# mormj/newsched

Measured on NVIDIA B200. Metric: Msamples/s FIR-ccf & FFT-4096 flowgraph at 1/2/4/8 B200; % of HBM/FP32 roofline, higher is better.
Workload: dtype f32

## Files before the change

### newsched_b200/csrc/common.cuh

```cuda
#pragma once
#include <cuda.h>
#include <cuda_runtime.h>
#include <atomic>
#include <cstdarg>
#include <cstdint>
#include <cstdio>
#include <cstring>

#include "../../include/b200dsp.h"

namespace b200 {

char* err_buf();
int set_err(int code, const char* fmt, ...);
extern std::atomic<int64_t> g_launches;

inline cudaStream_t cs(b200_stream_t s) { return reinterpret_cast<cudaStream_t>(s); }

#define B200_CUDA(call)                                                                  \
    do {                                                                                 \
        cudaError_t e__ = (call);                                                        \
        if (e__ != cudaSuccess)                                                          \
            return ::b200::set_err(B200_ERR_CUDA, "%s:%d %s -> %s", __FILE__, __LINE__,  \
                                   #call, cudaGetErrorString(e__));                      \
    } while (0)

#define B200_LAUNCH(kernel, grid, block, smem, stream, ...)                              \
    do {                                                                                 \
        kernel<<<(grid), (block), (smem), (stream)>>>(__VA_ARGS__);                      \
        ::b200::g_launches.fetch_add(1, std::memory_order_relaxed);                      \
        cudaError_t e__ = cudaPeekAtLastError();                                         \
        if (e__ != cudaSuccess)                                                          \
            return ::b200::set_err(B200_ERR_CUDA, "%s:%d launch %s -> %s", __FILE__,     \
                                   __LINE__, #kernel, cudaGetErrorString(e__));          \
    } while (0)

#define B200_LAUNCH_PDL(kernel, grid_, block_, smem_, stream_, ...)                          \
    do {                                                                                 \
        cudaLaunchConfig_t cfg__{};                                                      \
        cfg__.gridDim = dim3(grid_);                                                     \
        cfg__.blockDim = dim3(block_);                                                   \
        cfg__.dynamicSmemBytes = (smem_);                                                \
        cfg__.stream = (stream_);                                                        \
        cudaLaunchAttribute attr__[1];                                                   \
        attr__[0].id = cudaLaunchAttributeProgrammaticStreamSerialization;               \
        attr__[0].val.programmaticStreamSerializationAllowed = 1;                        \
        cfg__.attrs = attr__;                                                            \
        cfg__.numAttrs = 1;                                                              \
        cudaError_t e__ = cudaLaunchKernelEx(&cfg__, kernel, __VA_ARGS__);               \
        ::b200::g_launches.fetch_add(1, std::memory_order_relaxed);                      \
        if (e__ != cudaSuccess)                                                          \
            return ::b200::set_err(B200_ERR_CUDA, "%s:%d launch %s -> %s", __FILE__,     \
                                   __LINE__, #kernel, cudaGetErrorString(e__));          \
    } while (0)

__device__ __forceinline__ void pdl_wait() { asm volatile("griddepcontrol.wait;" ::: "memory"); }
__device__ __forceinline__ void pdl_launch_dependents() { asm volatile("griddepcontrol.launch_dependents;" ::: "memory"); }

int sm_count();

typedef CUresult (*tmap_encode_fn)(CUtensorMap*, CUtensorMapDataType, cuuint32_t, void*, const cuuint64_t*,
                                   const cuuint64_t*, const cuuint32_t*, const cuuint32_t*, CUtensorMapInterleave,
                                   CUtensorMapSwizzle, CUtensorMapL2promotion, CUtensorMapFloatOOBfill);
tmap_encode_fn tmap_encode_tiled();

__device__ __forceinline__ float2 cmul_nofma(float2 a, float kre, float kim)
{
    float ac = __fmul_rn(a.x, kre), bd = __fmul_rn(a.y, kim);
    float ad = __fmul_rn(a.x, kim), bc = __fmul_rn(a.y, kre);
    return make_float2(__fsub_rn(ac, bd), __fadd_rn(ad, bc));
}

#ifndef B200_PK_CMUL
#define B200_PK_CMUL 0
#endif
__device__ __forceinline__ float2 cmul(float2 a, float2 b)
{
#if B200_PK_CMUL
    const float2 r = __fmul2_rn(b, make_float2(a.x, a.x));
    return __ffma2_rn(make_float2(-b.y, b.x), make_float2(a.y, a.y), r);
#else
    return make_float2(fmaf(-a.y, b.y, a.x * b.x), fmaf(a.x, b.y, a.y * b.x));
#endif
}
__device__ __forceinline__ float2 cmul_conj(float2 a, float2 b)
{
#if B200_PK_CMUL
    const float2 r = __fmul2_rn(make_float2(b.x, -b.y), make_float2(a.x, a.x));
    return __ffma2_rn(make_float2(b.y, b.x), make_float2(a.y, a.y), r);
#else
    return make_float2(fmaf(a.y, b.y, a.x * b.x), fmaf(-a.x, b.y, a.y * b.x));
#endif
}
__device__ __forceinline__ float2 cmac(float2 a, float2 b, float2 acc)
{
#if B200_PK_CMUL
    acc = __ffma2_rn(b, make_float2(a.x, a.x), acc);
    return __ffma2_rn(make_float2(-b.y, b.x), make_float2(a.y, a.y), acc);
#else
    return make_float2(fmaf(a.x, b.x, fmaf(-a.y, b.y, acc.x)), fmaf(a.x, b.y, fmaf(a.y, b.x, acc.y)));
#endif
}

__device__ __forceinline__ float mag_nofma(float2 a)
{
    return __fsqrt_rn(__fadd_rn(__fmul_rn(a.x, a.x), __fmul_rn(a.y, a.y)));
}

__device__ __forceinline__ uint32_t smem_u32(const void* p)
{
    return (uint32_t)__cvta_generic_to_shared(p);
}
__device__ __forceinline__ void mbar_init(uint64_t* bar, uint32_t count)
{
    asm volatile("mbarrier.init.shared::cta.b64 [%0], %1;" ::"r"(smem_u32(bar)), "r"(count) : "memory");
}
__device__ __forceinline__ void fence_mbar_init()
{
    asm volatile("fence.mbarrier_init.release.cluster;" ::: "memory");
}
__device__ __forceinline__ void fence_proxy_async()
{
    asm volatile("fence.proxy.async.shared::cta;" ::: "memory");
}
__device__ __forceinline__ void mbar_arrive_expect_tx(uint64_t* bar, uint32_t bytes)
{
    asm volatile("mbarrier.arrive.expect_tx.shared::cta.b64 _, [%0], %1;" ::"r"(smem_u32(bar)), "r"(bytes)
                 : "memory");
}
__device__ __forceinline__ void bulk_copy_g2s(void* smem_dst, const void* gmem_src, uint32_t bytes,
                                              uint64_t* bar)
{
    asm volatile("cp.async.bulk.shared::cluster.global.mbarrier::complete_tx::bytes [%0], [%1], %2, [%3];" ::"r"(
                     smem_u32(smem_dst)),
                 "l"(gmem_src), "r"(bytes), "r"(smem_u32(bar))
                 : "memory");
}
__device__ __forceinline__ bool mbar_try_wait(uint64_t* bar, uint32_t parity)
{
    uint32_t ok;
    asm volatile("{\n"
                 ".reg .pred p;\n"
                 "mbarrier.try_wait.parity.shared::cta.b64 p, [%1], %2;\n"
                 "selp.u32 %0, 1, 0, p;\n"
                 "}"
                 : "=r"(ok)
                 : "r"(smem_u32(bar)), "r"(parity)
                 : "memory");
    return ok != 0;
}
__device__ __forceinline__ void mbar_wait(uint64_t* bar, uint32_t parity)
{
    for (uint32_t spins = 0; !mbar_try_wait(bar, parity); spins++)
        if (spins > (1u << 28))
            __trap();
}

}
```

### newsched_b200/csrc/fft.cu

```cuda
#include <cmath>
#include <cstdlib>
#include <vector>

#include "fft_core.cuh"

#ifndef B200_FFT_TW2
#define B200_FFT_TW2 1
#endif

namespace b200 {

template <bool FWD, int OUT>
__global__ void __launch_bounds__(256, 2)
    fft4096_kernel(const float2* __restrict__ in, void* __restrict__ out, long long n_vec,
                   const float* __restrict__ weff, const float2* __restrict__ tw1,
                   const float2* __restrict__ tw2)
{
    __shared__ float2 sA[16 * F4K_STRIDE];
    __shared__ float2 sT2[256];
    const int tid = threadIdx.x;

    float wreg[16];
    float2 t1[16];
#pragma unroll
    for (int i = 0; i < 16; i++) {
        wreg[i] = __ldg(weff + i * 256 + tid);
        t1[i] = __ldg(tw1 + i * 256 + tid);
    }
    sT2[tid] = __ldg(tw2 + tid);
    __syncthreads();

    for (long long vec = blockIdx.x; vec < n_vec; vec += gridDim.x) {
        const float2* x = in + vec * 4096;
        float2 v[16];
        if (tid == 0 && vec + gridDim.x < n_vec && ((uintptr_t)in % 16 == 0))
            asm volatile("cp.async.bulk.prefetch.L2.global [%0], %1;" ::"l"(in + (vec + gridDim.x) * 4096),
                         "r"(4096 * 8)
                         : "memory");
#pragma unroll
        for (int i = 0; i < 16; i++)
            v[i] = __ldcs(x + i * 256 + tid);
#pragma unroll
        for (int i = 0; i < 16; i++)
            v[i] = __fmul2_rn(v[i], make_float2(wreg[i], wreg[i]));
        dft16<FWD>(v);
#pragma unroll
        for (int k0 = 0; k0 < 16; k0++)
            sA[k0 * F4K_STRIDE + tid] = cmul(v[pos16(k0)], t1[k0]);
        __syncthreads();
        {
            const int k0 = tid >> 4, n0 = tid & 15;
            float2* row = sA + k0 * F4K_STRIDE + n0;
#pragma unroll
            for (int i = 0; i < 16; i++)
                v[i] = row[i * 16];
            dft16<FWD>(v);
            row[0] = v[pos16(0)];
#pragma unroll
            for (int k1 = 1; k1 < 16; k1++)
                row[k1 * 16] = cmul(v[pos16(k1)], sT2[k1 * 16 + n0]);
        }
        __syncthreads();
        {
            const int k0 = tid & 15, k1 = tid >> 4;
            const float2* row = sA + k0 * F4K_STRIDE + k1 * 16;
#pragma unroll
            for (int i = 0; i < 16; i++)
                v[i] = row[i];
            dft16<FWD>(v);
            if (OUT == B200_FFT_OUT_COMPLEX) {
                float2* y = reinterpret_cast<float2*>(out) + vec * 4096;
#pragma unroll
                for (int k2 = 0; k2 < 16; k2++)
                    __stcs(y + k2 * 256 + tid, v[pos16(k2)]);
            } else {
                float* y = reinterpret_cast<float*>(out) + vec * 4096;
#pragma unroll
                for (int k2 = 0; k2 < 16; k2++) {
                    float2 z = v[pos16(k2)];
                    float p = fmaf(z.x, z.x, z.y * z.y);
                    __stcs(y + k2 * 256 + tid, OUT == B200_FFT_OUT_MAG ? sqrt_approx(p) : p);
                }
            }
        }
        __syncthreads();
    }
}

constexpr int f4k_ntile(int out) { return out == B200_FFT_OUT_COMPLEX ? 2 : 3; }
constexpr size_t f4k_tma_smem(int out) { return (size_t)f4k_ntile(out) * (4096 * 8 + 8) + 256 * 8; }

__device__ __forceinline__ int f4k_swz(int n0, int k0) { return (((n0 >> 1) ^ (k0 & 7)) << 1) | (n0 & 1); }

template <bool FWD, int OUT>
__global__ void __launch_bounds__(256, 2)
    fft4096_tma_kernel(const float2* __restrict__ in, void* __restrict__ out, long long n_vec,
                       const float* __restrict__ weff, const float2* __restrict__ tw1,
                       const float2* __restrict__ tw2)
{
    constexpr int NT = f4k_ntile(OUT);
    extern __shared__ __align__(128) unsigned char smem_raw[];
    float2* sTile0 = reinterpret_cast<float2*>(smem_raw);
    float2* sT2 = sTile0 + 4096 * NT;
    uint64_t* bar0 = reinterpret_cast<uint64_t*>(sT2 + 256);
    const int tid = threadIdx.x;

    if (tid == 0) {
#pragma unroll
        for (int i = 0; i < NT; i++)
            mbar_init(bar0 + i, 1);
        fence_mbar_init();
    }
    float wreg[16];
    float2 t1[16];
#pragma unroll
    for (int i = 0; i < 16; i++) {
        wreg[i] = __ldg(weff + i * 256 + tid);
        t1[i] = __ldg(tw1 + i * 256 + tid);
    }
    sT2[tid] = __ldg(tw2 + tid);
    __syncthreads();
#if B200_FFT_TW2 == 1
    float2 t2r[16];
#pragma unroll
    for (int k1 = 1; k1 < 16; k1++)
        t2r[k1] = sT2[k1 * 16 + (tid & 15)];
#endif
    pdl_wait();
    pdl_launch_dependents();
    long long vec = blockIdx.x;
    if (tid == 0) {
#pragma unroll
        for (int i = 0; i < NT - 1; i++)
            if (vec + (long long)i * gridDim.x < n_vec) {
                mbar_arrive_expect_tx(bar0 + i, 4096 * 8);
                bulk_copy_g2s(sTile0 + 4096 * i, in + (vec + (long long)i * gridDim.x) * 4096, 4096 * 8, bar0 + i);
            }
    }
    int t = 0;
    uint32_t par = 0;
    for (; vec < n_vec; vec += gridDim.x) {
        float2 v[16];
        float2* tile = sTile0 + t * 4096;
        mbar_wait(bar0 + t, par);
#pragma unroll
        for (int i = 0; i < 16; i++)
            v[i] = tile[i * 256 + tid];
#pragma unroll
        for (int i = 0; i < 16; i++)
            v[i] = __fmul2_rn(v[i], make_float2(wreg[i], wreg[i]));
        dft16<FWD>(v);
#pragma unroll
        for (int k0 = 0; k0 < 16; k0++)
            tile[k0 * 256 + tid] = cmul(v[pos16(k0)], t1[k0]);
#if B200_FFT_TW2 == 2
        float2 t2r[16];
#pragma unroll
        for (int k1 = 1; k1 < 16; k1++)
            t2r[k1] = sT2[k1 * 16 + (tid & 15)];
#endif
        __syncthreads();
        const int tn = t == 0 ? NT - 1 : t - 1;
        if (tid == 0 && vec + (long long)(NT - 1) * gridDim.x < n_vec) {
            fence_proxy_async();
            mbar_arrive_expect_tx(bar0 + tn, 4096 * 8);
            bulk_copy_g2s(sTile0 + tn * 4096, in + (vec + (long long)(NT - 1) * gridDim.x) * 4096, 4096 * 8,
                          bar0 + tn);
        }
        {
            const int k0 = tid >> 4, n0 = tid & 15;
            float2* row = tile + k0 * 256;
#pragma unroll
            for (int i = 0; i < 16; i++)
                v[i] = row[i * 16 + n0];
            __syncwarp();
            dft16<FWD>(v);
            float2* dst = row + f4k_swz(n0, k0);
            dst[0] = v[pos16(0)];
#pragma unroll
            for (int k1 = 1; k1 < 16; k1++)
#if B200_FFT_TW2
                dst[k1 * 16] = cmul(v[pos16(k1)], t2r[k1]);
#else
                dst[k1 * 16] = cmul(v[pos16(k1)], sT2[k1 * 16 + n0]);
#endif
        }
        __syncthreads();
        {
            const int k0 = tid & 15, k1 = tid >> 4, s = k0 & 7;
            const float4* seg = reinterpret_cast<const float4*>(tile + k0 * 256 + k1 * 16);
#pragma unroll
            for (int j = 0; j < 8; j++) {
                const float4 q = seg[j ^ s];
                v[2 * j] = make_float2(q.x, q.y);
                v[2 * j + 1] = make_float2(q.z, q.w);
            }
            dft16<FWD>(v);
            if (OUT == B200_FFT_OUT_COMPLEX) {
                float2* y = reinterpret_cast<float2*>(out) + vec * 4096;
#pragma unroll
                for (int k2 = 0; k2 < 16; k2++)
                    __stcs(y + k2 * 256 + tid, v[pos16(k2)]);
            } else {
                float* y = reinterpret_cast<float*>(out) + vec * 4096;
#pragma unroll
                for (int k2 = 0; k2 < 16; k2++) {
                    float2 z = v[pos16(k2)];
                    float p = fmaf(z.x, z.x, z.y * z.y);
                    __stcs(y + k2 * 256 + tid, OUT == B200_FFT_OUT_MAG ? sqrt_approx(p) : p);
                }
            }
        }
        if (++t == NT) {
            t = 0;
            par ^= 1;
        }
    }
}

#ifndef B200_F8K_EARLY
#define B200_F8K_EARLY 0
#endif
constexpr size_t F8K_SMEM = 8192 * 8 + 16 * F4K_STRIDE * 8 + 256 * 8 + 32;

template <bool FWD, int I>
__device__ __forceinline__ float2 mul_w32(float2 z)
{
    constexpr double kPi = 3.14159265358979323846;
    constexpr float cr[16] = { 1.f, 0.98078528040323043f, 0.92387953251128674f, 0.83146961230254524f,
                               0.70710678118654752f, 0.55557023301960218f, 0.38268343236508977f,
                               0.19509032201612825f, 0.f, -0.19509032201612825f, -0.38268343236508977f,
                               -0.55557023301960218f, -0.70710678118654752f, -0.83146961230254524f,
                               -0.92387953251128674f, -0.98078528040323043f };
    constexpr float si[16] = { 0.f, 0.19509032201612825f, 0.38268343236508977f, 0.55557023301960218f,
                               0.70710678118654752f, 0.83146961230254524f, 0.92387953251128674f,
                               0.98078528040323043f, 1.f, 0.98078528040323043f, 0.92387953251128674f,
                               0.83146961230254524f, 0.70710678118654752f, 0.55557023301960218f,
                               0.38268343236508977f, 0.19509032201612825f };
    (void)kPi;
    if (I == 0)
        return z;
    constexpr float wr = cr[I], wi = FWD ? -si[I] : si[I];
    return make_float2(fmaf(-z.y, wi, z.x * wr), fmaf(z.x, wi, z.y * wr));
}

template <bool FWD, int I = 0>
__device__ __forceinline__ void f8k_split(float2 (&a)[16], float2* sIn, const float* __restrict__ w0,
                                          const float* __restrict__ w1, float2 wt, int tid)
{
    if constexpr (I < 16) {
        const float2 x0 = __fmul2_rn(sIn[I * 256 + tid], make_float2(w0[I], w0[I]));
        const float2 x1 = __fmul2_rn(sIn[4096 + I * 256 + tid], make_float2(w1[I], w1[I]));
        a[I] = x0 + x1;
        sIn[I * 256 + tid] = cmul(mul_w32<FWD, I>(x0 - x1), wt);
        f8k_split<FWD, I + 1>(a, sIn, w0, w1, wt, tid);
    }
}

template <bool FWD, int OUT>
__global__ void __launch_bounds__(256, 2)
    fft8192_kernel(const float2* __restrict__ in, void* __restrict__ out, long long n_vec,
                   const float* __restrict__ weff, const float2* __restrict__ tw1,
                   const float2* __restrict__ tw2, float odd_sign)
{
    extern __shared__ __align__(128) unsigned char smem_raw[];
    float2* sIn = reinterpret_cast<float2*>(smem_raw);
    float2* sA = sIn + 8192;
    float2* sT2 = sA + 16 * F4K_STRIDE;
    uint64_t* bar = reinterpret_cast<uint64_t*>(sT2 + 256);
    const int tid = threadIdx.x;
    if (tid == 0) {
        mbar_init(bar, 1);
        mbar_init(bar + 1, 1);
        fence_mbar_init();
    }
    float2 t1[16];
#pragma unroll
    for (int i = 0; i < 16; i++)
        t1[i] = __ldg(tw1 + i * 256 + tid);
    sT2[tid] = __ldg(tw2 + tid);
    float2 wt;
    {
        float sn, cs_;
        sincospif((float)tid / 4096.0f, &sn, &cs_);
        wt = make_float2(cs_ * odd_sign, (FWD ? -sn : sn) * odd_sign);
    }
    __syncthreads();
    pdl_wait();
    pdl_launch_dependents();
    long long vec = blockIdx.x;
    if (tid == 0 && vec < n_vec) {
        mbar_arrive_expect_tx(bar, 4096 * 8);
        bulk_copy_g2s(sIn, in + vec * 8192, 4096 * 8, bar);
        mbar_arrive_expect_tx(bar + 1, 4096 * 8);
        bulk_copy_g2s(sIn + 4096, in + vec * 8192 + 4096, 4096 * 8, bar + 1);
    }
    uint32_t phase = 0;
    for (; vec < n_vec; vec += gridDim.x) {
        float2 e[16], v[16];
        {
            float w0[16], w1[16];
#pragma unroll
            for (int i = 0; i < 16; i++) {
                w0[i] = __ldg(weff + i * 256 + tid);
                w1[i] = __ldg(weff + 4096 + i * 256 + tid);
            }
            mbar_wait(bar, phase);
            mbar_wait(bar + 1, phase);
            phase ^= 1;
            f8k_split<FWD>(e, sIn, w0, w1, wt, tid);
        }
        dft16<FWD>(e);
#pragma unroll
        for (int k0 = 0; k0 < 16; k0++)
            sA[k0 * F4K_STRIDE + tid] = cmul(e[pos16(k0)], t1[k0]);
        __syncthreads();
        const long long nxt = vec + gridDim.x;
        if (tid == 0 && nxt < n_vec) {
            mbar_arrive_expect_tx(bar + 1, 4096 * 8);
            bulk_copy_g2s(sIn + 4096, in + nxt * 8192 + 4096, 4096 * 8, bar + 1);
        }
        {
            const int k0 = tid >> 4, n0 = tid & 15;
            float2* row = sA + k0 * F4K_STRIDE + n0;
#pragma unroll
            for (int i = 0; i < 16; i++)
                e[i] = row[i * 16];
            dft16<FWD>(e);
            row[0] = e[pos16(0)];
#pragma unroll
            for (int k1 = 1; k1 < 16; k1++)
                row[k1 * 16] = cmul(e[pos16(k1)], sT2[k1 * 16 + n0]);
        }
        __syncthreads();
        {
            const int k0 = tid & 15, k1 = tid >> 4;
            const float2* row = sA + k0 * F4K_STRIDE + k1 * 16;
#pragma unroll
            for (int i = 0; i < 16; i++)
                e[i] = row[i];
            dft16<FWD>(e);
        }
#if B200_F8K_EARLY
        if (OUT == B200_FFT_OUT_COMPLEX) {
            float2* y = reinterpret_cast<float2*>(out) + vec * 8192;
#pragma unroll
            for (int k2 = 0; k2 < 16; k2++)
                __stcs(y + 2 * (k2 * 256 + tid), e[pos16(k2)]);
        } else {
            float* y = reinterpret_cast<float*>(out) + vec * 8192;
#pragma unroll
            for (int k2 = 0; k2 < 16; k2++) {
                const float2 p = e[pos16(k2)];
                const float pe = fmaf(p.x, p.x, p.y * p.y);
                __stcs(y + 2 * (k2 * 256 + tid), OUT == B200_FFT_OUT_MAG ? sqrt_approx(pe) : pe);
            }
        }
#endif
        __syncthreads();
#pragma unroll
        for (int i = 0; i < 16; i++)
            v[i] = sIn[i * 256 + tid];
        dft16<FWD>(v);
#pragma unroll
        for (int k0 = 0; k0 < 16; k0++)
            sA[k0 * F4K_STRIDE + tid] = cmul(v[pos16(k0)], t1[k0]);
        __syncthreads();
        if (tid == 0 && nxt < n_vec) {
            mbar_arrive_expect_tx(bar, 4096 * 8);
            bulk_copy_g2s(sIn, in + nxt * 8192, 4096 * 8, bar);
// ... 296 lines not shown
            for (int i = 0; i < 16; i++)
                v[i] = row[i];
            dft16<FWD>(v);
            const int vv = tid / R0, k0 = tid % R0;
            float2* orow = sO + vv * G::OS + k0;
#pragma unroll
            for (int k1 = 0; k1 < 16; k1++)
                orow[k1 * R0] = v[pos16(k1)];
        }
        __syncthreads();
#pragma unroll
        for (int i = 0; i < 16; i++) {
            const int e = i * 256 + tid;
            const int vv = e / G::N, k = e % G::N;
            if (vec0 + vv < n_vec) {
                float2 z = sO[vv * G::OS + k];
                if (OUT == B200_FFT_OUT_COMPLEX) {
                    if (flip && (k & 1))
                        z = make_float2(-z.x, -z.y);
                    __stcs(reinterpret_cast<float2*>(out) + blk * 4096 + e, z);
                } else {
                    float p = fmaf(z.x, z.x, z.y * z.y);
                    __stcs(reinterpret_cast<float*>(out) + blk * 4096 + e, OUT == B200_FFT_OUT_MAG ? sqrt_approx(p) : p);
                }
            }
        }
        __syncthreads();
    }
}

template <bool FWD, int OUT>
__global__ void __launch_bounds__(256)
    fft8_kernel(const float2* __restrict__ in, void* __restrict__ out, long long n_vec,
                const float* __restrict__ weff, float2 post, int flip)
{
    float w[8];
#pragma unroll
    for (int i = 0; i < 8; i++)
        w[i] = __ldg(weff + i);
    const long long stride = (long long)gridDim.x * blockDim.x;
    for (long long v = (long long)blockIdx.x * blockDim.x + threadIdx.x; v < n_vec; v += stride) {
        const float4* src = reinterpret_cast<const float4*>(in + v * 8);
        float2 z[8];
#pragma unroll
        for (int i = 0; i < 4; i++) {
            const float4 t = __ldcs(src + i);
            z[2 * i] = make_float2(t.x * w[2 * i], t.y * w[2 * i]);
            z[2 * i + 1] = make_float2(t.z * w[2 * i + 1], t.w * w[2 * i + 1]);
        }
        dft8<FWD>(z);
        if (OUT == B200_FFT_OUT_COMPLEX) {
#pragma unroll
            for (int k = 0; k < 8; k++) {
                z[k] = cmul(z[k], post);
                if (flip && (k & 1))
                    z[k] = make_float2(-z[k].x, -z[k].y);
            }
            float4* dst = reinterpret_cast<float4*>(out) + v * 4;
#pragma unroll
            for (int i = 0; i < 4; i++)
                __stcs(dst + i, make_float4(z[2 * i].x, z[2 * i].y, z[2 * i + 1].x, z[2 * i + 1].y));
        } else {
            float m[8];
#pragma unroll
            for (int k = 0; k < 8; k++) {
                const float pw = fmaf(z[k].x, z[k].x, z[k].y * z[k].y);
                m[k] = OUT == B200_FFT_OUT_MAG ? sqrt_approx(pw) : pw;
            }
            float4* dst = reinterpret_cast<float4*>(out) + v * 2;
            __stcs(dst, make_float4(m[0], m[1], m[2], m[3]));
            __stcs(dst + 1, make_float4(m[4], m[5], m[6], m[7]));
        }
    }
}

template <bool FWD, int OUT>
__global__ void __launch_bounds__(512)
    fft_generic_kernel(const float2* __restrict__ in, void* __restrict__ out, long long n_vec, int N,
                       int log2n, int vpb, const float* __restrict__ weff,
                       const float2* __restrict__ tw, float2 post, int flip)
{
    extern __shared__ __align__(16) float2 sbuf[];
    const int per_cta = vpb * N;
    float2* bx = sbuf;
    float2* by = sbuf + per_cta;
    const long long v0 = (long long)blockIdx.x * vpb;
    const int nv = (int)((n_vec - v0) < vpb ? (n_vec - v0) : vpb);
    if (nv <= 0)
        return;
    const int tot = nv * N;
    const float2* x = in + v0 * N;
    for (int i = threadIdx.x; i < tot; i += blockDim.x) {
        float2 t = __ldcs(x + i);
        float w = __ldg(weff + (i & (N - 1)));
        bx[i] = make_float2(t.x * w, t.y * w);
    }
    __syncthreads();
    const int half = N >> 1;
    int s_log = 0;
    for (int n_log = log2n; n_log >= 1; n_log--, s_log++) {
        const int m = 1 << (n_log - 1);
        const int s = 1 << s_log;
        for (int i = threadIdx.x; i < nv * half; i += blockDim.x) {
            int vi = i / half;
            int bi = i - vi * half;
            int p = bi >> s_log;
            int q = bi & (s - 1);
            const float2* xb = bx + vi * N;
            float2* yb = by + vi * N;
            float2 a = xb[q + s * p];
            float2 b = xb[q + s * (p + m)];
            float2 w = __ldg(tw + (p << (log2n - n_log)));
            float2 d = a - b;
            yb[q + s * 2 * p] = a + b;
            yb[q + s * (2 * p + 1)] = cmul(d, w);
        }
        __syncthreads();
        float2* t = bx;
        bx = by;
        by = t;
    }
    for (int i = threadIdx.x; i < tot; i += blockDim.x) {
        float2 z = bx[i];
        int k = i & (N - 1);
        if (OUT == B200_FFT_OUT_COMPLEX) {
            z = cmul(z, post);
            if (flip && (k & 1))
                z = make_float2(-z.x, -z.y);
            __stcs(reinterpret_cast<float2*>(out) + v0 * N + i, z);
        } else {
            float pw = fmaf(z.x, z.x, z.y * z.y);
            __stcs(reinterpret_cast<float*>(out) + v0 * N + i,
                   OUT == B200_FFT_OUT_MAG ? sqrt_approx(pw) : pw);
        }
    }
}

}

using namespace b200;

struct b200_fft {
    int N = 0, log2n = 0;
    int forward = 1, out_mode = 0;
    int flip = 0;
    float2 post{ 1.f, 0.f };
    float* d_weff = nullptr;
    float2* d_tw1 = nullptr;
    float2* d_tw2 = nullptr;
    float2* d_tw = nullptr;
    int vpb = 1;
    int grid_4k = 296;
    int use_tma = 1;
};

template <bool FWD, int OUT>
static int fft_run_t(b200_fft* h, const void* d_in, void* d_out, long long n_vec, cudaStream_t s)
{
    if (h->N == 4096) {
        long long g = n_vec < h->grid_4k ? n_vec : h->grid_4k;
        if (h->use_tma && (uintptr_t)d_in % 16 == 0)
            B200_LAUNCH_PDL((fft4096_tma_kernel<FWD, OUT>), (unsigned)g, 256, f4k_tma_smem(OUT), s,
                        (const float2*)d_in, d_out, n_vec, h->d_weff, h->d_tw1, h->d_tw2);
        else
            B200_LAUNCH((fft4096_kernel<FWD, OUT>), (unsigned)g, 256, 0, s, (const float2*)d_in, d_out,
                        n_vec, h->d_weff, h->d_tw1, h->d_tw2);
    } else if (h->N == 16 || h->N == 32 || h->N == 64 || h->N == 128) {
        const int R0 = h->N / 16, V = 4096 / h->N;
        long long nb = (n_vec + V - 1) / V;
        long long g = nb < h->grid_4k ? nb : h->grid_4k;
        const int tma_ok = (uintptr_t)d_in % 16 == 0;
#define FFT_SM_GO(R)                                                                                     \
    B200_LAUNCH_PDL((fft_small_kernel<R, FWD, OUT>), (unsigned)g, 256, fsm<R>::SMEM, s, (const float2*)d_in, \
                d_out, n_vec, h->d_weff, h->d_tw1, h->flip, tma_ok)
        switch (R0) {
        case 1: FFT_SM_GO(1); break;
        case 2: FFT_SM_GO(2); break;
        case 4: FFT_SM_GO(4); break;
        default: FFT_SM_GO(8); break;
        }
#undef FFT_SM_GO
    } else if (h->N == 256 || h->N == 512 || h->N == 1024 || h->N == 2048) {
        const int R0 = h->N / 256, V = 16 / R0;
        long long nb = (n_vec + V - 1) / V;
        long long g = nb < h->grid_4k ? nb : h->grid_4k;
        const int tma_ok = (uintptr_t)d_in % 16 == 0;
#define FFT_R0_GO(R)                                                                                  \
    B200_LAUNCH_PDL((fft_r0_kernel<R, FWD, OUT>), (unsigned)g, 256, fr0<R>::SMEM, s, (const float2*)d_in, \
                d_out, n_vec, h->d_weff, h->d_tw1, h->d_tw2, tma_ok)
        switch (R0) {
        case 1: FFT_R0_GO(1); break;
        case 2: FFT_R0_GO(2); break;
        case 4: FFT_R0_GO(4); break;
        default: FFT_R0_GO(8); break;
        }
#undef FFT_R0_GO
    } else if (h->N == 8 && (uintptr_t)d_in % 16 == 0 && (uintptr_t)d_out % 16 == 0) {
        long long blocks = (n_vec + 255) / 256;
        const long long cap = 16LL * sm_count();
        B200_LAUNCH((fft8_kernel<FWD, OUT>), (unsigned)(blocks < cap ? blocks : cap), 256, 0, s, (const float2*)d_in,
                    d_out, n_vec, h->d_weff, h->post, h->flip);
    } else if (h->N == 8192 && h->d_tw1 && (uintptr_t)d_in % 16 == 0 && (uintptr_t)d_out % 16 == 0) {
        long long g = n_vec < h->grid_4k ? n_vec : h->grid_4k;
        B200_LAUNCH_PDL((fft8192_kernel<FWD, OUT>), (unsigned)g, 256, F8K_SMEM, s, (const float2*)d_in, d_out, n_vec,
                    h->d_weff, h->d_tw1, h->d_tw2, h->flip ? -1.f : 1.f);
    } else {
        long long blocks = (n_vec + h->vpb - 1) / h->vpb;
        if (blocks > 0x7fffffffLL)
            return set_err(B200_ERR_ARG, "fft: too many vectors for one call");
        int work = h->vpb * h->N / 2;
        int nt = work < 512 ? (work < 32 ? 32 : work) : 512;
        size_t smem = sizeof(float2) * 2 * (size_t)h->vpb * h->N;
        B200_LAUNCH((fft_generic_kernel<FWD, OUT>), (unsigned)blocks, nt, smem, s,
                    (const float2*)d_in, d_out, n_vec, h->N, h->log2n, h->vpb, h->d_weff, h->d_tw,
                    h->post, h->flip);
    }
    return B200_OK;
}

template <bool FWD>
static int fft_run_o(b200_fft* h, const void* d_in, void* d_out, long long n_vec, cudaStream_t s)
{
    switch (h->out_mode) {
    case B200_FFT_OUT_COMPLEX:
        return fft_run_t<FWD, B200_FFT_OUT_COMPLEX>(h, d_in, d_out, n_vec, s);
    case B200_FFT_OUT_MAG:
        return fft_run_t<FWD, B200_FFT_OUT_MAG>(h, d_in, d_out, n_vec, s);
    default:
        return fft_run_t<FWD, B200_FFT_OUT_MAG_SQUARED>(h, d_in, d_out, n_vec, s);
    }
}

template <bool FWD, int OUT>
static cudaError_t fft_tma_attr()
{
    return cudaFuncSetAttribute(fft4096_tma_kernel<FWD, OUT>,
                                cudaFuncAttributeMaxDynamicSharedMemorySize, (int)f4k_tma_smem(OUT));
}

template <int R0, bool FWD, int OUT>
static cudaError_t fft_r0_attr()
{
    return cudaFuncSetAttribute(fft_r0_kernel<R0, FWD, OUT>, cudaFuncAttributeMaxDynamicSharedMemorySize,
                                (int)fr0<R0>::SMEM);
}
template <int R0>
static cudaError_t fft_r0_attr_all()
{
    cudaError_t e = cudaSuccess;
    if ((e = fft_r0_attr<R0, true, 0>()) != cudaSuccess) return e;
    if ((e = fft_r0_attr<R0, true, 1>()) != cudaSuccess) return e;
    if ((e = fft_r0_attr<R0, true, 2>()) != cudaSuccess) return e;
    if ((e = fft_r0_attr<R0, false, 0>()) != cudaSuccess) return e;
    if ((e = fft_r0_attr<R0, false, 1>()) != cudaSuccess) return e;
    return fft_r0_attr<R0, false, 2>();
}

template <int R0, bool FWD, int OUT>
static cudaError_t fft_small_attr()
{
    return cudaFuncSetAttribute(fft_small_kernel<R0, FWD, OUT>, cudaFuncAttributeMaxDynamicSharedMemorySize,
                                (int)fsm<R0>::SMEM);
}
template <int R0>
static cudaError_t fft_small_attr_all()
{
    cudaError_t e = cudaSuccess;
    if ((e = fft_small_attr<R0, true, 0>()) != cudaSuccess) return e;
    if ((e = fft_small_attr<R0, true, 1>()) != cudaSuccess) return e;
    if ((e = fft_small_attr<R0, true, 2>()) != cudaSuccess) return e;
    if ((e = fft_small_attr<R0, false, 0>()) != cudaSuccess) return e;
    if ((e = fft_small_attr<R0, false, 1>()) != cudaSuccess) return e;
    return fft_small_attr<R0, false, 2>();
}

template <bool FWD, int OUT>
static cudaError_t fft_generic_attr()
{
    return cudaFuncSetAttribute(fft_generic_kernel<FWD, OUT>,
                                cudaFuncAttributeMaxDynamicSharedMemorySize, 160 * 1024);
}

extern "C" {

int b200_fft_destroy(b200_fft* h)
{
    if (!h)
        return B200_OK;
    cudaFree(h->d_weff);
    cudaFree(h->d_tw1);
    cudaFree(h->d_tw2);
    cudaFree(h->d_tw);
    delete h;
    return B200_OK;
}

int b200_fft_create(const b200_fft_params* p, b200_fft** out)
{
    if (!p || !out)
        return set_err(B200_ERR_ARG, "fft_create: null argument");
    *out = nullptr;
    const int N = p->n;
    if (N < 8 || N > 8192 || (N & (N - 1)))
        return set_err(B200_ERR_UNSUPPORTED, "fft_create: N must be a power of two in [8, 8192], got %d", N);
    if (p->output < 0 || p->output > 2)
        return set_err(B200_ERR_ARG, "fft_create: bad output mode %d", p->output);
    b200_fft* h = new b200_fft();
    h->N = N;
    while ((1 << h->log2n) < N)
        h->log2n++;
    h->forward = p->forward ? 1 : 0;
    h->out_mode = p->output;
    const double sgn = h->forward ? -1.0 : 1.0;

    double kmag = 1.0, kph_re = 1.0, kph_im = 0.0;
    if (p->fuse_pre_multiply_const) {
        kmag = std::hypot((double)p->k_re, (double)p->k_im);
        if (kmag > 0.0) {
            kph_re = p->k_re / kmag;
            kph_im = p->k_im / kmag;
        }
    }
    std::vector<float> weff(N);
    for (int n = 0; n < N; n++) {
        double w;
        if (!h->forward && p->shift) {
            w = p->window ? (double)p->window[(n + N - N / 2) % N] : 1.0;
        } else {
            w = p->window ? (double)p->window[n] : 1.0;
            if (h->forward && p->shift && (n & 1))
                w = -w;
        }
        weff[n] = (float)(w * kmag);
    }
    h->flip = (!h->forward && p->shift) ? 1 : 0;
    h->post = make_float2((float)kph_re, (float)kph_im);

#define FFT_CUDA(call)                                                                   \
    do {                                                                                 \
        cudaError_t e__ = (call);                                                        \
        if (e__ != cudaSuccess) {                                                        \
            b200_fft_destroy(h);                                                         \
            return set_err(e__ == cudaErrorMemoryAllocation ? B200_ERR_NOMEM : B200_ERR_CUDA, \
                           "fft_create: %s -> %s", #call, cudaGetErrorString(e__));      \
        }                                                                                \
    } while (0)

    FFT_CUDA(cudaMalloc(&h->d_weff, sizeof(float) * N));
    FFT_CUDA(cudaMemcpy(h->d_weff, weff.data(), sizeof(float) * N, cudaMemcpyHostToDevice));
    if (N == 4096) {
        std::vector<float2> t1(16 * 256), t2(256);
        for (int k0 = 0; k0 < 16; k0++)
            for (int L = 0; L < 256; L++) {
                double ang = sgn * 2.0 * M_PI * (double)((L * k0) % 4096) / 4096.0;
                double wr = std::cos(ang), wi = std::sin(ang);
                double pr = kph_re, pi = kph_im;
                if (h->flip && (k0 & 1)) {
                    pr = -pr;
                    pi = -pi;
                }
                t1[k0 * 256 + L] = make_float2((float)(wr * pr - wi * pi), (float)(wr * pi + wi * pr));
            }
        for (int k1 = 0; k1 < 16; k1++)
            for (int n0 = 0; n0 < 16; n0++) {
                double ang = sgn * 2.0 * M_PI * (double)(n0 * k1) / 256.0;
                t2[k1 * 16 + n0] = make_float2((float)std::cos(ang), (float)std::sin(ang));
            }
        FFT_CUDA(cudaMalloc(&h->d_tw1, sizeof(float2) * t1.size()));
        FFT_CUDA(cudaMemcpy(h->d_tw1, t1.data(), sizeof(float2) * t1.size(), cudaMemcpyHostToDevice));
        FFT_CUDA(cudaMalloc(&h->d_tw2, sizeof(float2) * t2.size()));
        FFT_CUDA(cudaMemcpy(h->d_tw2, t2.data(), sizeof(float2) * t2.size(), cudaMemcpyHostToDevice));
        h->grid_4k = 2 * sm_count();
        if (const char* e = getenv("B200_FFT_TMA"))
            h->use_tma = atoi(e);
        if (const char* e = getenv("B200_FFT_GRID_PER_SM"))
            h->grid_4k = atoi(e) * sm_count();
        FFT_CUDA((fft_tma_attr<true, 0>()));
        FFT_CUDA((fft_tma_attr<true, 1>()));
        FFT_CUDA((fft_tma_attr<true, 2>()));
        FFT_CUDA((fft_tma_attr<false, 0>()));
        FFT_CUDA((fft_tma_attr<false, 1>()));
        FFT_CUDA((fft_tma_attr<false, 2>()));
    } else if (N == 16 || N == 32 || N == 64 || N == 128) {
        const int R0 = N / 16;
        std::vector<float2> t1((size_t)R0 * 16);
        for (int k0 = 0; k0 < R0; k0++)
            for (int n0 = 0; n0 < 16; n0++) {
                double ang = sgn * 2.0 * M_PI * (double)(n0 * k0) / (double)N;
                double wr = std::cos(ang), wi = std::sin(ang);
                t1[(size_t)k0 * 16 + n0] =
                    make_float2((float)(wr * kph_re - wi * kph_im), (float)(wr * kph_im + wi * kph_re));
            }
        FFT_CUDA(cudaMalloc(&h->d_tw1, sizeof(float2) * 128));
        FFT_CUDA(cudaMemset(h->d_tw1, 0, sizeof(float2) * 128));
        FFT_CUDA(cudaMemcpy(h->d_tw1, t1.data(), sizeof(float2) * t1.size(), cudaMemcpyHostToDevice));
        h->grid_4k = 2 * sm_count();
        FFT_CUDA(fft_small_attr_all<1>());
        FFT_CUDA(fft_small_attr_all<2>());
        FFT_CUDA(fft_small_attr_all<4>());
        FFT_CUDA(fft_small_attr_all<8>());
    } else if (N == 256 || N == 512 || N == 1024 || N == 2048) {
        const int R0 = N / 256;
        std::vector<float2> t1((size_t)R0 * 256), t2(256);
        for (int k0 = 0; k0 < R0; k0++)
            for (int L = 0; L < 256; L++) {
                double ang = sgn * 2.0 * M_PI * (double)((L * k0) % N) / (double)N;
                double wr = std::cos(ang), wi = std::sin(ang);
                double pr = kph_re, pi = kph_im;
                if (h->flip && R0 > 1 && (k0 & 1)) {
                    pr = -pr;
                    pi = -pi;
                }
                t1[(size_t)k0 * 256 + L] = make_float2((float)(wr * pr - wi * pi), (float)(wr * pi + wi * pr));
            }
        for (int k1 = 0; k1 < 16; k1++)
            for (int n0 = 0; n0 < 16; n0++) {
                double ang = sgn * 2.0 * M_PI * (double)(n0 * k1) / 256.0;
                double f = (h->flip && R0 == 1 && (k1 & 1)) ? -1.0 : 1.0;
                t2[k1 * 16 + n0] = make_float2((float)(f * std::cos(ang)), (float)(f * std::sin(ang)));
            }
        FFT_CUDA(cudaMalloc(&h->d_tw1, sizeof(float2) * t1.size()));
        FFT_CUDA(cudaMemcpy(h->d_tw1, t1.data(), sizeof(float2) * t1.size(), cudaMemcpyHostToDevice));
        FFT_CUDA(cudaMalloc(&h->d_tw2, sizeof(float2) * t2.size()));
        FFT_CUDA(cudaMemcpy(h->d_tw2, t2.data(), sizeof(float2) * t2.size(), cudaMemcpyHostToDevice));
        h->grid_4k = 2 * sm_count();
        FFT_CUDA(fft_r0_attr_all<1>());
        FFT_CUDA(fft_r0_attr_all<2>());
        FFT_CUDA(fft_r0_attr_all<4>());
        FFT_CUDA(fft_r0_attr_all<8>());
    } else {
        std::vector<float2> tw(N / 2);
        for (int j = 0; j < N / 2; j++) {
            double ang = sgn * 2.0 * M_PI * (double)j / (double)N;
            tw[j] = make_float2((float)std::cos(ang), (float)std::sin(ang));
        }
        FFT_CUDA(cudaMalloc(&h->d_tw, sizeof(float2) * tw.size()));
        FFT_CUDA(cudaMemcpy(h->d_tw, tw.data(), sizeof(float2) * tw.size(), cudaMemcpyHostToDevice));
        h->vpb = N >= 1024 ? 1 : 1024 / N;
        FFT_CUDA((fft_generic_attr<true, 0>()));
        FFT_CUDA((fft_generic_attr<true, 1>()));
        FFT_CUDA((fft_generic_attr<true, 2>()));
        FFT_CUDA((fft_generic_attr<false, 0>()));
        FFT_CUDA((fft_generic_attr<false, 1>()));
        FFT_CUDA((fft_generic_attr<false, 2>()));
        if (N == 8192 && !getenv("B200_FFT_GENERIC")) {
            std::vector<float2> t1(16 * 256), t2(256);
            for (int k0 = 0; k0 < 16; k0++)
                for (int L = 0; L < 256; L++) {
                    double ang = sgn * 2.0 * M_PI * (double)((L * k0) % 4096) / 4096.0;
                    double wr = std::cos(ang), wi = std::sin(ang);
                    t1[k0 * 256 + L] =
                        make_float2((float)(wr * kph_re - wi * kph_im), (float)(wr * kph_im + wi * kph_re));
                }
            for (int k1 = 0; k1 < 16; k1++)
                for (int n0 = 0; n0 < 16; n0++) {
                    double ang = sgn * 2.0 * M_PI * (double)(n0 * k1) / 256.0;
                    t2[k1 * 16 + n0] = make_float2((float)std::cos(ang), (float)std::sin(ang));
                }
            FFT_CUDA(cudaMalloc(&h->d_tw1, sizeof(float2) * t1.size()));
            FFT_CUDA(cudaMemcpy(h->d_tw1, t1.data(), sizeof(float2) * t1.size(), cudaMemcpyHostToDevice));
            FFT_CUDA(cudaMalloc(&h->d_tw2, sizeof(float2) * t2.size()));
            FFT_CUDA(cudaMemcpy(h->d_tw2, t2.data(), sizeof(float2) * t2.size(), cudaMemcpyHostToDevice));
            h->grid_4k = 2 * sm_count();
#define F8K_ATTR(FW, O) \
    FFT_CUDA(cudaFuncSetAttribute(fft8192_kernel<FW, O>, cudaFuncAttributeMaxDynamicSharedMemorySize, (int)F8K_SMEM))
            F8K_ATTR(true, 0);
            F8K_ATTR(true, 1);
            F8K_ATTR(true, 2);
            F8K_ATTR(false, 0);
            F8K_ATTR(false, 1);
            F8K_ATTR(false, 2);
#undef F8K_ATTR
        }
    }
#undef FFT_CUDA
    if (cudaDeviceSynchronize() != cudaSuccess) {
        b200_fft_destroy(h);
        return set_err(B200_ERR_CUDA, "fft_create: %s", cudaGetErrorString(cudaGetLastError()));
    }
    *out = h;
    return B200_OK;
}

int b200_fft_geometry(const b200_fft* h, int* n, int* out_item_bytes)
{
    if (!h)
        return set_err(B200_ERR_ARG, "fft_geometry: null handle");
    if (n)
        *n = h->N;
    if (out_item_bytes)
        *out_item_bytes = h->out_mode == B200_FFT_OUT_COMPLEX ? 8 : 4;
    return B200_OK;
}

int b200_fft_run(b200_fft* h, const void* d_in, void* d_out, int64_t n_vectors, b200_stream_t s)
{
    if (!h || n_vectors < 0 || (n_vectors > 0 && (!d_in || !d_out)))
        return set_err(B200_ERR_ARG, "fft_run: bad argument");
    if (n_vectors == 0)
        return B200_OK;
    if ((uintptr_t)d_in % 8 || (uintptr_t)d_out % (h->out_mode == B200_FFT_OUT_COMPLEX ? 8 : 4))
        return set_err(B200_ERR_ARG, "fft_run: misaligned buffer");
    return h->forward ? fft_run_o<true>(h, d_in, d_out, n_vectors, cs(s))
                      : fft_run_o<false>(h, d_in, d_out, n_vectors, cs(s));
}

}
```

Measured before the change: 512,800.

## Use cluster launch control work-stealing for complex-output 4096-point FFT kernel

For complex output, the TMA FFT-4096 kernel now launches one CTA per vector and uses Blackwell cluster launch control (try_cancel) to claim not-yet-started CTAs' vectors as work. Persistent CTAs prefetch claimed vectors into a shared-memory ring via bulk copies. This replaces the fixed grid-stride loop with dynamic scheduling, aimed at better load balance and at letting the hardware scheduler hand out work. It adds an mbarrier round-trip per tile and a dependency of the prefetch chain on claim latency.

```diff
diff --git a/newsched_b200/csrc/common.cuh b/newsched_b200/csrc/common.cuh
--- a/newsched_b200/csrc/common.cuh
+++ b/newsched_b200/csrc/common.cuh
@@ -156,4 +156,29 @@
             __trap();
 }
 
+__device__ __forceinline__ void clc_try_cancel(void* resp, uint64_t* bar)
+{
+    mbar_arrive_expect_tx(bar, 16);
+    asm volatile("clusterlaunchcontrol.try_cancel.async.shared::cta.mbarrier::complete_tx::bytes.b128 [%0], [%1];" ::"r"(
+                     smem_u32(resp)),
+                 "r"(smem_u32(bar))
+                 : "memory");
 }
+__device__ __forceinline__ int clc_cancelled_ctaid_x(const void* resp)
+{
+    int x;
+    asm volatile("{\n"
+                 ".reg .b128 r;\n"
+                 ".reg .pred p;\n"
+                 "ld.shared.b128 r, [%1];\n"
+                 "mov.s32 %0, -1;\n"
+                 "clusterlaunchcontrol.query_cancel.is_canceled.pred.b128 p, r;\n"
+                 "@p clusterlaunchcontrol.query_cancel.get_first_ctaid::x.b32.b128 %0, r;\n"
+                 "}"
+                 : "=r"(x)
+                 : "r"(smem_u32(resp))
+                 : "memory");
+    return x;
+}
+
+}
diff --git a/newsched_b200/csrc/fft.cu b/newsched_b200/csrc/fft.cu
--- a/newsched_b200/csrc/fft.cu
+++ b/newsched_b200/csrc/fft.cu
@@ -88,7 +88,16 @@
 }
 
 constexpr int f4k_ntile(int out) { return out == B200_FFT_OUT_COMPLEX ? 2 : 3; }
-constexpr size_t f4k_tma_smem(int out) { return (size_t)f4k_ntile(out) * (4096 * 8 + 8) + 256 * 8; }
+constexpr bool f4k_claims(int out) { return out == B200_FFT_OUT_COMPLEX; }
+constexpr size_t f4k_resp_off(int out)
+{
+    return ((size_t)f4k_ntile(out) * 4096 * 8 + 256 * 8 + (f4k_ntile(out) + 1) * 8 + 15) / 16 * 16;
+}
+constexpr size_t f4k_tma_smem(int out)
+{
+    return f4k_claims(out) ? f4k_resp_off(out) + 16 + f4k_ntile(out) * 4
+                           : (size_t)f4k_ntile(out) * (4096 * 8 + 8) + 256 * 8;
+}
 
 __device__ __forceinline__ int f4k_swz(int n0, int k0) { return (((n0 >> 1) ^ (k0 & 7)) << 1) | (n0 & 1); }
 
@@ -99,17 +108,25 @@
                        const float2* __restrict__ tw2)
 {
     constexpr int NT = f4k_ntile(OUT);
+    constexpr bool CLAIM = f4k_claims(OUT);
     extern __shared__ __align__(128) unsigned char smem_raw[];
     float2* sTile0 = reinterpret_cast<float2*>(smem_raw);
     float2* sT2 = sTile0 + 4096 * NT;
     uint64_t* bar0 = reinterpret_cast<uint64_t*>(sT2 + 256);
+    uint64_t* cbar = bar0 + NT;
+    void* sResp = smem_raw + f4k_resp_off(OUT);
+    int* sVec = reinterpret_cast<int*>(smem_raw + f4k_resp_off(OUT) + 16);
     const int tid = threadIdx.x;
 
     if (tid == 0) {
 #pragma unroll
         for (int i = 0; i < NT; i++)
             mbar_init(bar0 + i, 1);
+        if (CLAIM)
+            mbar_init(cbar, 1);
         fence_mbar_init();
+        if (CLAIM)
+            clc_try_cancel(sResp, cbar);
     }
     float wreg[16];
     float2 t1[16];
@@ -129,17 +146,39 @@
     pdl_wait();
     pdl_launch_dependents();
     long long vec = blockIdx.x;
+    uint32_t cpar = 0;
+    bool claiming = true;
+    auto take_claimed = [&](int tile) {
+        int cv = -1;
+        if (claiming) {
+            mbar_wait(cbar, cpar);
+            cpar ^= 1;
+            cv = clc_cancelled_ctaid_x(sResp);
+        }
+        if (cv >= 0) {
+            fence_proxy_async();
+            mbar_arrive_expect_tx(bar0 + tile, 4096 * 8);
+            bulk_copy_g2s(sTile0 + tile * 4096, in + (long long)cv * 4096, 4096 * 8, bar0 + tile);
+            clc_try_cancel(sResp, cbar);
+        } else {
+            claiming = false;
+        }
+        sVec[tile] = cv;
+    };
     if (tid == 0) {
 #pragma unroll
-        for (int i = 0; i < NT - 1; i++)
-            if (vec + (long long)i * gridDim.x < n_vec) {
+        for (int i = 0; i < NT - 1; i++) {
+            if (CLAIM && i > 0) {
+                take_claimed(i);
+            } else if (vec + (long long)i * gridDim.x < n_vec) {
                 mbar_arrive_expect_tx(bar0 + i, 4096 * 8);
                 bulk_copy_g2s(sTile0 + 4096 * i, in + (vec + (long long)i * gridDim.x) * 4096, 4096 * 8, bar0 + i);
             }
+        }
     }
     int t = 0;
     uint32_t par = 0;
-    for (; vec < n_vec; vec += gridDim.x) {
+    while (CLAIM || vec < n_vec) {
         float2 v[16];
         float2* tile = sTile0 + t * 4096;
         mbar_wait(bar0 + t, par);
@@ -161,7 +200,10 @@
 #endif
         __syncthreads();
         const int tn = t == 0 ? NT - 1 : t - 1;
-        if (tid == 0 && vec + (long long)(NT - 1) * gridDim.x < n_vec) {
+        if (CLAIM) {
+            if (tid == 0)
+                take_claimed(tn);
+        } else if (tid == 0 && vec + (long long)(NT - 1) * gridDim.x < n_vec) {
             fence_proxy_async();
             mbar_arrive_expect_tx(bar0 + tn, 4096 * 8);
             bulk_copy_g2s(sTile0 + tn * 4096, in + (vec + (long long)(NT - 1) * gridDim.x) * 4096, 4096 * 8,
@@ -214,6 +256,13 @@
         if (++t == NT) {
             t = 0;
             par ^= 1;
+        }
+        if (CLAIM) {
+            vec = sVec[t];
+            if (vec < 0)
+                break;
+        } else {
+            vec += gridDim.x;
         }
     }
 }
@@ -825,12 +874,18 @@
 {
     if (h->N == 4096) {
         long long g = n_vec < h->grid_4k ? n_vec : h->grid_4k;
-        if (h->use_tma && (uintptr_t)d_in % 16 == 0)
+        if (h->use_tma && (uintptr_t)d_in % 16 == 0) {
+            if (f4k_claims(OUT)) {
+                if (n_vec > 0x7fffffffLL)
+                    return set_err(B200_ERR_ARG, "fft: too many vectors for one call");
+                g = n_vec;
+            }
             B200_LAUNCH_PDL((fft4096_tma_kernel<FWD, OUT>), (unsigned)g, 256, f4k_tma_smem(OUT), s,
-                        (const float2*)d_in, d_out, n_vec, h->d_weff, h->d_tw1, h->d_tw2);
-        else
+                            (const float2*)d_in, d_out, n_vec, h->d_weff, h->d_tw1, h->d_tw2);
+        } else {
             B200_LAUNCH((fft4096_kernel<FWD, OUT>), (unsigned)g, 256, 0, s, (const float2*)d_in, d_out,
                         n_vec, h->d_weff, h->d_tw1, h->d_tw2);
+        }
     } else if (h->N == 16 || h->N == 32 || h->N == 64 || h->N == 128) {
         const int R0 = h->N / 16, V = 4096 / h->N;
         long long nb = (n_vec + V - 1) / V;
```

Measured after the change: 513,400, median of 6. Within noise of the previous version (+0.1%).

## Use dynamic atomic work-stealing for FFT-4096 TMA kernel and prefetch first tiles to L2

Applied to the files above, without the earlier changes.

Replaces the static grid-stride vector assignment in the TMA FFT-4096 kernel with a per-launch global atomic counter, so each CTA claims its next vector dynamically. The aim is to balance load across CTAs and remove tail imbalance. It also issues L2 bulk prefetches for the first tiles before barrier setup, and adds an optional compile-time timeline instrumentation path. The cost is one atomic per vector on thread 0, a shared-memory vector index array, and a rotating pool of scheduler slots that assumes no more than 256 launches are in flight at once.

```diff
diff --git a/newsched_b200/csrc/fft.cu b/newsched_b200/csrc/fft.cu
--- a/newsched_b200/csrc/fft.cu
+++ b/newsched_b200/csrc/fft.cu
@@ -88,7 +88,30 @@
 }
 
 constexpr int f4k_ntile(int out) { return out == B200_FFT_OUT_COMPLEX ? 2 : 3; }
-constexpr size_t f4k_tma_smem(int out) { return (size_t)f4k_ntile(out) * (4096 * 8 + 8) + 256 * 8; }
+constexpr size_t f4k_tma_smem(int out) { return (size_t)f4k_ntile(out) * (4096 * 8 + 16) + 256 * 8; }
+
+struct f4k_sched {
+    unsigned long long next;
+    unsigned int done;
+    unsigned int pad;
+};
+constexpr int F4K_SCHED_SLOTS = 256;
+
+#ifdef B200_FFT_TIMELINE
+struct f4k_tl_rec {
+    unsigned long long t_start, t_end;
+    unsigned int smid, n_vec;
+};
+constexpr int F4K_TL_LAUNCHES = 64, F4K_TL_CTAS = 512;
+__device__ f4k_tl_rec g_f4k_tl[F4K_TL_LAUNCHES * F4K_TL_CTAS];
+__device__ unsigned long long g_f4k_tl_seq;
+__device__ __forceinline__ unsigned long long f4k_globaltimer()
+{
+    unsigned long long t;
+    asm volatile("mov.u64 %0, %%globaltimer;" : "=l"(t));
+    return t;
+}
+#endif
 
 __device__ __forceinline__ int f4k_swz(int n0, int k0) { return (((n0 >> 1) ^ (k0 & 7)) << 1) | (n0 & 1); }
 
@@ -96,16 +119,23 @@
 __global__ void __launch_bounds__(256, 2)
     fft4096_tma_kernel(const float2* __restrict__ in, void* __restrict__ out, long long n_vec,
                        const float* __restrict__ weff, const float2* __restrict__ tw1,
-                       const float2* __restrict__ tw2)
+                       const float2* __restrict__ tw2, f4k_sched* __restrict__ sched)
 {
     constexpr int NT = f4k_ntile(OUT);
     extern __shared__ __align__(128) unsigned char smem_raw[];
     float2* sTile0 = reinterpret_cast<float2*>(smem_raw);
     float2* sT2 = sTile0 + 4096 * NT;
     uint64_t* bar0 = reinterpret_cast<uint64_t*>(sT2 + 256);
+    long long* sVec = reinterpret_cast<long long*>(bar0 + NT);
     const int tid = threadIdx.x;
 
     if (tid == 0) {
+#pragma unroll
+        for (int i = 0; i < NT - 1; i++) {
+            const long long v = blockIdx.x + (long long)i * gridDim.x;
+            if (v < n_vec)
+                asm volatile("cp.async.bulk.prefetch.L2.global [%0], %1;" ::"l"(in + v * 4096), "r"(4096 * 8) : "memory");
+        }
 #pragma unroll
         for (int i = 0; i < NT; i++)
             mbar_init(bar0 + i, 1);
@@ -128,18 +158,31 @@
 #endif
     pdl_wait();
     pdl_launch_dependents();
-    long long vec = blockIdx.x;
+#ifdef B200_FFT_TIMELINE
+    unsigned long long tl_seq = 0, tl_start = 0;
+    unsigned int tl_n = 0;
     if (tid == 0) {
-#pragma unroll
-        for (int i = 0; i < NT - 1; i++)
-            if (vec + (long long)i * gridDim.x < n_vec) {
+        tl_start = f4k_globaltimer();
+        tl_seq = atomicAdd(&g_f4k_tl_seq, 1ull);
+    }
+#endif
+    long long nxt = 0;
+    if (tid == 0) {
+#pragma unroll
+        for (int i = 0; i < NT - 1; i++) {
+            const long long v = blockIdx.x + (long long)i * gridDim.x;
+            if (v < n_vec) {
                 mbar_arrive_expect_tx(bar0 + i, 4096 * 8);
-                bulk_copy_g2s(sTile0 + 4096 * i, in + (vec + (long long)i * gridDim.x) * 4096, 4096 * 8, bar0 + i);
-            }
-    }
+                bulk_copy_g2s(sTile0 + 4096 * i, in + v * 4096, 4096 * 8, bar0 + i);
+            }
+            sVec[i] = v < n_vec ? v : -1;
+        }
+        nxt = (long long)(NT - 1) * gridDim.x + (sched ? (long long)atomicAdd(&sched->next, 1ull) : blockIdx.x);
+    }
+    __syncthreads();
     int t = 0;
     uint32_t par = 0;
-    for (; vec < n_vec; vec += gridDim.x) {
+    while (sVec[t] >= 0) {
         float2 v[16];
         float2* tile = sTile0 + t * 4096;
         mbar_wait(bar0 + t, par);
@@ -161,11 +204,17 @@
 #endif
         __syncthreads();
         const int tn = t == 0 ? NT - 1 : t - 1;
-        if (tid == 0 && vec + (long long)(NT - 1) * gridDim.x < n_vec) {
-            fence_proxy_async();
-            mbar_arrive_expect_tx(bar0 + tn, 4096 * 8);
-            bulk_copy_g2s(sTile0 + tn * 4096, in + (vec + (long long)(NT - 1) * gridDim.x) * 4096, 4096 * 8,
-                          bar0 + tn);
+        if (tid == 0) {
+            if (nxt < n_vec) {
+                fence_proxy_async();
+                mbar_arrive_expect_tx(bar0 + tn, 4096 * 8);
+                bulk_copy_g2s(sTile0 + tn * 4096, in + nxt * 4096, 4096 * 8, bar0 + tn);
+                sVec[tn] = nxt;
+                nxt = sched ? (long long)(NT - 1) * gridDim.x + (long long)atomicAdd(&sched->next, 1ull)
+                            : nxt + gridDim.x;
+            } else {
+                sVec[tn] = -1;
+            }
         }
         {
             const int k0 = tid >> 4, n0 = tid & 15;
@@ -197,12 +246,12 @@
             }
             dft16<FWD>(v);
             if (OUT == B200_FFT_OUT_COMPLEX) {
-                float2* y = reinterpret_cast<float2*>(out) + vec * 4096;
+                float2* y = reinterpret_cast<float2*>(out) + sVec[t] * 4096;
 #pragma unroll
                 for (int k2 = 0; k2 < 16; k2++)
                     __stcs(y + k2 * 256 + tid, v[pos16(k2)]);
             } else {
-                float* y = reinterpret_cast<float*>(out) + vec * 4096;
+                float* y = reinterpret_cast<float*>(out) + sVec[t] * 4096;
 #pragma unroll
                 for (int k2 = 0; k2 < 16; k2++) {
                     float2 z = v[pos16(k2)];
@@ -215,7 +264,28 @@
             t = 0;
             par ^= 1;
         }
-    }
+#ifdef B200_FFT_TIMELINE
+        tl_n++;
+#endif
+    }
+    if (sched && tid == 0) {
+        __threadfence();
+        if (atomicAdd(&sched->done, 1u) == gridDim.x - 1) {
+            sched->next = 0;
+            sched->done = 0;
+        }
+    }
+#ifdef B200_FFT_TIMELINE
+    if (tid == 0 && blockIdx.x < F4K_TL_CTAS) {
+        f4k_tl_rec& r = g_f4k_tl[(tl_seq / gridDim.x) % F4K_TL_LAUNCHES * F4K_TL_CTAS + blockIdx.x];
+        unsigned int smid;
+        asm volatile("mov.u32 %0, %%smid;" : "=r"(smid));
+        r.t_start = tl_start;
+        r.t_end = f4k_globaltimer();
+        r.smid = smid;
+        r.n_vec = tl_n;
+    }
+#endif
 }
 
 #ifndef B200_F8K_EARLY
@@ -818,6 +888,8 @@
     int vpb = 1;
     int grid_4k = 296;
     int use_tma = 1;
+    f4k_sched* d_sched = nullptr;
+    std::atomic<unsigned int> sched_seq{ 0 };
 };
 
 template <bool FWD, int OUT>
@@ -825,10 +897,13 @@
 {
     if (h->N == 4096) {
         long long g = n_vec < h->grid_4k ? n_vec : h->grid_4k;
-        if (h->use_tma && (uintptr_t)d_in % 16 == 0)
+        if (h->use_tma && (uintptr_t)d_in % 16 == 0) {
+            f4k_sched* sc = h->d_sched ? h->d_sched + h->sched_seq.fetch_add(1, std::memory_order_relaxed) %
+                                                          F4K_SCHED_SLOTS
+                                       : nullptr;
             B200_LAUNCH_PDL((fft4096_tma_kernel<FWD, OUT>), (unsigned)g, 256, f4k_tma_smem(OUT), s,
-                        (const float2*)d_in, d_out, n_vec, h->d_weff, h->d_tw1, h->d_tw2);
-        else
+                        (const float2*)d_in, d_out, n_vec, h->d_weff, h->d_tw1, h->d_tw2, sc);
+        } else
             B200_LAUNCH((fft4096_kernel<FWD, OUT>), (unsigned)g, 256, 0, s, (const float2*)d_in, d_out,
                         n_vec, h->d_weff, h->d_tw1, h->d_tw2);
     } else if (h->N == 16 || h->N == 32 || h->N == 64 || h->N == 128) {
@@ -957,6 +1032,7 @@
     cudaFree(h->d_tw1);
     cudaFree(h->d_tw2);
     cudaFree(h->d_tw);
+    cudaFree(h->d_sched);
     delete h;
     return B200_OK;
 }
@@ -1041,6 +1117,11 @@
             h->use_tma = atoi(e);
         if (const char* e = getenv("B200_FFT_GRID_PER_SM"))
             h->grid_4k = atoi(e) * sm_count();
+        const char* sched = getenv("B200_FFT_SCHED");
+        if (!sched || strcmp(sched, "static") != 0) {
+            FFT_CUDA(cudaMalloc(&h->d_sched, sizeof(f4k_sched) * F4K_SCHED_SLOTS));
+            FFT_CUDA(cudaMemset(h->d_sched, 0, sizeof(f4k_sched) * F4K_SCHED_SLOTS));
+        }
         FFT_CUDA((fft_tma_attr<true, 0>()));
         FFT_CUDA((fft_tma_attr<true, 1>()));
         FFT_CUDA((fft_tma_attr<true, 2>()));
@@ -1171,4 +1252,25 @@
                       : fft_run_o<false>(h, d_in, d_out, n_vectors, cs(s));
 }
 
-}
+#ifdef B200_FFT_TIMELINE
+B200_API int b200_fft_timeline_read(void* host, int64_t capacity_bytes, int64_t* ctas, int reset)
+{
+    if (!host || !ctas || capacity_bytes < (int64_t)sizeof(g_f4k_tl))
+        return set_err(B200_ERR_ARG, "fft_timeline_read: need %zu bytes", sizeof(g_f4k_tl));
+    unsigned long long seq = 0;
+    B200_CUDA(cudaMemcpyFromSymbol(host, g_f4k_tl, sizeof(g_f4k_tl)));
+    B200_CUDA(cudaMemcpyFromSymbol(&seq, g_f4k_tl_seq, sizeof(seq)));
+    *ctas = (int64_t)seq;
+    if (reset) {
+        void* p = nullptr;
+        B200_CUDA(cudaGetSymbolAddress(&p, g_f4k_tl));
+        B200_CUDA(cudaMemset(p, 0, sizeof(g_f4k_tl)));
+        seq = 0;
+        B200_CUDA(cudaMemcpyToSymbol(g_f4k_tl_seq, &seq, sizeof(seq)));
+        B200_CUDA(cudaDeviceSynchronize());
+    }
+    return B200_OK;
+}
+#endif
+
+}
```

Result: faster. 511,800 before, 522,300 after, median of 6 (+2.1%).
